# gaozhitong/MultiShiftSeg

Measured on AMD Instinct MI355X. Metric: train images/sec (DeepLabV3+ WRN38, fwd + RelContrastiveLoss + bwd + Adam), higher is better.
Workload: dtype f32; 1 GPU; c3: 2 images (1 orig+aug pair(s)) of 1024x2048 per GPU, stage-2 trainable set, train-mode BN/Dropout2d on the frozen trunk; images_per_gpu=2, height=1024, width=2048, stage=2, parallelism=dp1, rccl_ranks=0, loss_pairing=device, loss_sync=local

## Files before the change

### multishiftseg_amd/csrc/conv_wgrad.hip

```cpp
#include "mss_epilogue.h"
#include "wgrad_route.h"
static_assert(MSS_WGRAD_PERIMG_TAIL_BYTES == (long long)TN_PERIMG_MAX_SLOTS * 128 * 128 * 4, "include/mss_hip.h and tn_perimg_plan.h disagree");
#include <stdlib.h>

bool mss_wgrad_tn_bf16x3_eligible(const MssConvArgs& p, int lddy);
long long mss_wgrad_tn_bf16x3_ws_bytes(const MssConvArgs& p, int Cp);
void mss_wgrad_tn_bf16x3_plan(const MssConvArgs& p, WgradRoute& r);
int mss_wgrad_tn_bf16x3_launch(const MssConvArgs& p, const float* dy, int lddy, float* dwp, int Cp, float* ws, long long ws_bytes, void* stream);
int mss_stem7_wgrad_launch(const WgradRoute& r, const MssConvArgs& p, const float* dy, int lddy, float* dwp, float* ws, hipStream_t stream);

namespace {

constexpr int NT = 256;

template <int BKO, int BCI, int BP, int WK>
__global__ __launch_bounds__(NT) void conv_wgrad_kernel(MssConvArgs p, const float* __restrict__ dy, int lddy,
                                                        float* __restrict__ dwp, int Cp, int pix_per_split) {
  constexpr int LDA = BKO + 4;
  constexpr int LDB = BCI + 4;
  constexpr int WC = 4 / WK;
  constexpr int WTK = BKO / WK, WTC = BCI / WC;
  constexpr int TM = WTK / 32, TN = WTC / 32;
  constexpr int A_CPR = BKO / 4, B_CPR = BCI / 4;
  constexpr bool A_PART = BP * A_CPR < NT;
// ... 439 lines not shown
  };
  f32x16 acc[2][TNJ];
  auto zero_acc = [&]() {
#pragma unroll
    for (int i = 0; i < 2; ++i)
#pragma unroll
      for (int j = 0; j < TNJ; ++j)
#pragma unroll
        for (int q = 0; q < 16; ++q) acc[i][j][q] = 0.f;
  };
  auto mfma_chunk = [&](int set) {
#pragma unroll
    for (int s2 = 0; s2 < 4; ++s2)
#pragma unroll
      for (int i = 0; i < 2; ++i)
#pragma unroll
        for (int j = 0; j < TNJ; ++j)
          acc[i][j] = __builtin_amdgcn_mfma_f32_32x32x2f32(fa[set][i][s2], fb[set][j][s2], acc[i][j], 0, 0, 0);
  };
  auto epilogue = [&](long long w) {
    const int ct = (int)(w % ctiles); w /= ctiles;
    const int kt = (int)(w % ktiles); w /= ktiles;
    float* o = dst + (size_t)w * Kpad * Cp;
    const int colq = lane & 31, rowq = 4 * (lane >> 5);
#pragma unroll
    for (int j = 0; j < TNJ; ++j) {
      const int col = ct * BC + wn * (BC / 2) + j * 32 + colq;
      if (col >= Cp) continue;
#pragma unroll
      for (int i = 0; i < 2; ++i)
#pragma unroll
        for (int q = 0; q < 16; ++q) {
          const int row = kt * 128 + wm * 64 + i * 32 + (q & 3) + 8 * (q >> 2) + rowq;
          if (row < Kpad) o[(size_t)row * Cp + col] = acc[i][j][q];
        }
    }
  };

  long long cur = ld_w;
  int steps_left;
  {
    long long w = cur / ((long long)ktiles * ctiles);
    const int sp = (int)(w / P);
    const int t0 = sp * t_per_split;
    steps_left = (min(T, t0 + t_per_split) - t0 + 15) / 16;
  }
  setup(ld_w);
  issue_loads();
  finish_store(0);
  advance();
  zero_acc();
  __syncthreads();
  load_frags(0, 0, 0);
  int buf = 0;
  while (true) {
    issue_loads();
    load_frags(1, buf, 1);
    finish_store(buf ^ 1);
    advance();
    mfma_chunk(0);
    __syncthreads();
    load_frags(0, buf ^ 1, 0);
    mfma_chunk(1);
    buf ^= 1;
    if (--steps_left == 0) {
      epilogue(cur);
      cur += stride;
      if (cur >= total) break;
      zero_acc();
      long long w = cur / ((long long)ktiles * ctiles);
      const int sp = (int)(w / P);
      const int t0 = sp * t_per_split;
      steps_left = (min(T, t0 + t_per_split) - t0 + 15) / 16;
    }
  }
}

__global__ __launch_bounds__(256) void wgrad_reduce_kernel(const float* __restrict__ ws, float* __restrict__ dwp,
                                                           long long slab4, int splits) {
  const f32x4* w4 = reinterpret_cast<const f32x4*>(ws);
  f32x4* d4 = reinterpret_cast<f32x4*>(dwp);
  for (long long i = (long long)blockIdx.x * blockDim.x + threadIdx.x; i < slab4;
       i += (long long)gridDim.x * blockDim.x) {
    f32x4 a = w4[i];
    int sp = 1;
    for (; sp + 8 <= splits; sp += 8) {
      f32x4 v[8];
#pragma unroll
      for (int u = 0; u < 8; ++u) v[u] = w4[(long long)(sp + u) * slab4 + i];
#pragma unroll
      for (int u = 0; u < 8; ++u) a += v[u];
    }
    for (; sp < splits; ++sp) a += w4[(long long)sp * slab4 + i];
    d4[i] = a;
  }
}

template <int G>
__global__ __launch_bounds__(256) void wgrad_reduce_par_kernel(const float* __restrict__ ws, float* __restrict__ dwp, long long slab4,
                                                               int splits) {
  constexpr int EPB = 256 / G;
  __shared__ f32x4 part[G][EPB];
  const f32x4* w4 = reinterpret_cast<const f32x4*>(ws);
  const int el = threadIdx.x % EPB, g = threadIdx.x / EPB;
  const long long i = (long long)blockIdx.x * EPB + el;
  f32x4 a = {0.f, 0.f, 0.f, 0.f};
  if (i < slab4) {
    int sp = g;
    for (; sp + 3 * G < splits; sp += 4 * G) {
      const f32x4 v0 = w4[(long long)sp * slab4 + i], v1 = w4[(long long)(sp + G) * slab4 + i];
      const f32x4 v2 = w4[(long long)(sp + 2 * G) * slab4 + i], v3 = w4[(long long)(sp + 3 * G) * slab4 + i];
      a += v0; a += v1; a += v2; a += v3;
    }
    for (; sp < splits; sp += G) a += w4[(long long)sp * slab4 + i];
  }
  part[g][el] = a;
  __syncthreads();
  if (g == 0 && i < slab4) {
    f32x4 t = part[0][el];
#pragma unroll
    for (int k = 1; k < G; ++k) t += part[k][el];
    reinterpret_cast<f32x4*>(dwp)[i] = t;
  }
}

inline void launch_wgrad_reduce(const float* ws, float* dwp, long long slab4, int splits, int G, hipStream_t stream) {
  if (G == 1) {
    long long blocks = (slab4 + 255) / 256;
    if (blocks > 4096) blocks = 4096;
    hipLaunchKernelGGL(wgrad_reduce_kernel, dim3((int)blocks), dim3(256), 0, stream, ws, dwp, slab4, splits);
    return;
  }
#define RED(G_) hipLaunchKernelGGL(wgrad_reduce_par_kernel<G_>, dim3((unsigned)((slab4 + 256 / G_ - 1) / (256 / G_))), dim3(256), 0, stream, ws, dwp, slab4, splits)
  switch (G) {
    case 2: RED(2); break;
    case 4: RED(4); break;
    case 8: RED(8); break;
    case 16: RED(16); break;
    default: RED(32); break;
  }
#undef RED
}

typedef float f32x2 __attribute__((ext_vector_type(2)));
__device__ const float tn_zero_row[4096] = {0.f};
template <bool AFFINE = false, bool PERIMG = false>
__global__ __launch_bounds__(256, 1) void gemm_tn_direct_kernel(const float* __restrict__ A, const float* __restrict__ B,
                                                                float* __restrict__ out, int P, int M, int K, int C, long long a_bs,
                                                                long long b_bs, int Kpad, int Cp, int ktiles, int ctiles, int splits,
                                                                int tps, long long total, long long full, float* __restrict__ tail_ws,
                                                                const float* __restrict__ scale = nullptr,
                                                                const float* __restrict__ shift = nullptr, int relu = 0, int lda = 0,
                                                                const int* __restrict__ k_steps = nullptr, int k_base = 0,
                                                                int k_imgs = 1, int pi_slots = 0) {
  if (lda <= 0) lda = K;
  constexpr int KB = 4;
  constexpr int TND = 8;
  const int lane = threadIdx.x & 63, wave = threadIdx.x >> 6;
  long long t;
  int sp = 0, nsp = 1;
  long long tail_tile = -1, ntail = 0;
  int ct, kt, pb;
  if (PERIMG && pi_slots > 0) {
    const TnPerimgPlan pl = tn_perimg_plan(P / k_imgs, k_imgs, ktiles, ctiles, k_base, k_steps, pi_slots, M, tail_ws != nullptr);
    const int nwg = (int)((pl.total + 3) / 4), nrun = pl.tail ? (int)(pl.full / 4) : nwg;
    const int bid = (int)blockIdx.x;
    if (bid >= nwg) return;
    const long long job = (long long)(bid < nrun ? mss_xcd_remap(bid, nrun) : bid) * 4 + __builtin_amdgcn_readfirstlane(wave);
    TnPerimgJob jb;
    if (!tn_perimg_decode(pl, k_steps, job, jb)) return;
    ct = jb.ct; kt = jb.kt; pb = jb.pos * k_imgs + jb.img;
    if (jb.tail_tile >= 0) { sp = jb.sp; nsp = pl.splits; tail_tile = jb.tail_tile; ntail = pl.tail; tps = pl.tps; }
  } else {
    const long long job = (long long)(PERIMG ? mss_xcd_remap((int)blockIdx.x, (int)gridDim.x) : (int)blockIdx.x) * 4 + wave;
    if (job >= total) return;
    t = job;
    if (full >= 0) {
      if (job >= full) {
        ntail = (total - full) / splits;
        sp = (int)((job - full) / ntail);
        tail_tile = (job - full) - (long long)sp * ntail;
        t = full + tail_tile;
        nsp = splits;
      }
    } else {
      nsp = splits;
    }
    ct = (int)(t % ctiles); t /= ctiles;
    kt = (int)(t % ktiles); t /= ktiles;
    if (full >= 0) pb = (int)t;
    else { sp = (int)(t % splits); pb = (int)(t / splits); }
  }
  const int half = lane >> 5, j = lane & 31;
  const int r0 = nsp > 1 ? sp * tps : 0, r1 = nsp > 1 ? (r0 + tps < M ? r0 + tps : M) : M;
  const float* a = A + (size_t)pb * a_bs + (size_t)(kt * (32 * KB) + KB * j);
  const float* b = B + (size_t)pb * b_bs + (size_t)(ct * 128 + 4 * j);
  size_t b_ld = (size_t)C;
  if (PERIMG) {
    const int cend = 16 * (k_base + k_steps[pb % k_imgs]);
    if (ct * 128 >= cend) return;
    if (ct * 128 + 4 * j >= cend) { b = tn_zero_row + 4 * j; b_ld = 0; }
  }
  f32x16 acc[KB][4];
#pragma unroll
  for (int i = 0; i < KB; ++i)
#pragma unroll
    for (int q = 0; q < 4; ++q)
#pragma unroll
      for (int r = 0; r < 16; ++r) acc[i][q][r] = 0.f;
  f32x4 a0[TND], a1[TND];
  f32x4 b0[TND], b1[TND];
  const int last = r1 - 1;
  const float* az = tn_zero_row + (kt * (32 * KB) + KB * j);
  auto fetch = [&](int row, f32x4& va, f32x4& vb) {
    const bool ok = row <= last;
    const size_t rr = (size_t)(ok ? row : last);
    va = *reinterpret_cast<const f32x4*>(ok ? a + rr * lda : az);
    vb = *reinterpret_cast<const f32x4*>(b + rr * (PERIMG ? b_ld : (size_t)C));
  };
  f32x4 sc = {1.f, 1.f, 1.f, 1.f}, sh = {0.f, 0.f, 0.f, 0.f};
  if (AFFINE) {
    if (scale) sc = *reinterpret_cast<const f32x4*>(scale + ct * 128 + 4 * j);
    if (shift) sh = *reinterpret_cast<const f32x4*>(shift + ct * 128 + 4 * j);
  }
  const float fl = relu ? 0.f : -__builtin_huge_valf();
  auto compute = [&](const f32x4 (&va)[TND], const f32x4 (&vb)[TND]) {
#pragma unroll
    for (int d = 0; d < TND; ++d) {
      const f32x4 ca = va[d];
      f32x4 cb = vb[d];
      if (AFFINE) {
        cb = cb * sc + sh;
        cb.x = fmaxf(cb.x, fl); cb.y = fmaxf(cb.y, fl); cb.z = fmaxf(cb.z, fl); cb.w = fmaxf(cb.w, fl);
      }
#pragma unroll
      for (int i = 0; i < KB; ++i)
#pragma unroll
        for (int q = 0; q < 4; ++q) acc[i][q] = __builtin_amdgcn_mfma_f32_32x32x2f32(ca[i], cb[q], acc[i][q], 0, 0, 0);
    }
  };
#pragma unroll
  for (int d = 0; d < TND; ++d) fetch(r0 + 2 * d + half, a0[d], b0[d]);
  for (int r = r0; r < r1; r += 4 * TND) {
#pragma unroll
    for (int d = 0; d < TND; ++d) fetch(r + 2 * TND + 2 * d + half, a1[d], b1[d]);
    __builtin_amdgcn_sched_barrier(0);
    compute(a0, b0);
    __builtin_amdgcn_sched_barrier(0);
#pragma unroll
    for (int d = 0; d < TND; ++d) fetch(r + 4 * TND + 2 * d + half, a0[d], b0[d]);
    __builtin_amdgcn_sched_barrier(0);
    compute(a1, b1);
    __builtin_amdgcn_sched_barrier(0);
  }
  float* o;
  size_t ostride;
  if (tail_tile >= 0) {
    o = tail_ws + ((size_t)sp * ntail + tail_tile) * (128 * 128) + (size_t)(4 * j);
    ostride = 128;
  } else {
    o = out + ((size_t)(full >= 0 ? 0 : sp) * P + pb) * Kpad * Cp + (size_t)(kt * (32 * KB)) * Cp + (size_t)(ct * 128 + 4 * j);
    ostride = Cp;
  }
#pragma unroll
  for (int i = 0; i < KB; ++i)
#pragma unroll
    for (int r = 0; r < 16; ++r) {
      const int m = (r & 3) + 8 * (r >> 2) + 4 * half;
      const f32x4 v = {acc[i][0][r], acc[i][1][r], acc[i][2][r], acc[i][3][r]};
      *reinterpret_cast<f32x4*>(o + (size_t)(KB * m + i) * ostride) = v;
    }
}

__global__ __launch_bounds__(256) void tn_tail_reduce_kernel(const float* __restrict__ tail_ws, float* __restrict__ dwp, long long full,
                                                             long long ntail, int splits, int ktiles, int ctiles, int Kpad, int Cp) {
  const long long ti = blockIdx.x / 16;
  const int part = blockIdx.x % 16;
  long long t = full + ti;
  const int ct = (int)(t % ctiles); t /= ctiles;
  const int kt = (int)(t % ktiles); t /= ktiles;
  const int pb = (int)t;
  const int e = part * 1024 + threadIdx.x * 4;
  const int row = e >> 7, col = e & 127;
  const float* src = tail_ws + (size_t)ti * (128 * 128) + e;
  f32x4 a = *reinterpret_cast<const f32x4*>(src);
  for (int sp = 1; sp < splits; ++sp) a += *reinterpret_cast<const f32x4*>(src + (size_t)sp * ntail * (128 * 128));
  *reinterpret_cast<f32x4*>(dwp + (size_t)pb * Kpad * Cp + (size_t)(kt * 128 + row) * Cp + ct * 128 + col) = a;
}

__global__ __launch_bounds__(256) void tn_tail_reduce_perimg_kernel(const float* __restrict__ tail_ws, float* __restrict__ dwp, int P,
                                                                    int k_imgs, int ktiles, int ctiles, int k_base,
                                                                    const int* __restrict__ k_steps, int slots, int rows, int Kpad,
                                                                    int Cp) {
  const int ti = blockIdx.x / 16, part = blockIdx.x % 16;
  const TnPerimgPlan pl = tn_perimg_plan(P, k_imgs, ktiles, ctiles, k_base, k_steps, slots, rows, 1);
  if (ti >= pl.tail) return;
  TnPerimgJob jb;
  if (!tn_perimg_decode(pl, k_steps, pl.full + ti, jb)) return;
  const int pb = jb.pos * k_imgs + jb.img;
  const int e = part * 1024 + threadIdx.x * 4;
  const int row = e >> 7, col = e & 127;
  const float* src = tail_ws + (size_t)ti * (128 * 128) + e;
  f32x4 a = *reinterpret_cast<const f32x4*>(src);
  for (int sp = 1; sp < pl.splits; ++sp) a += *reinterpret_cast<const f32x4*>(src + (size_t)sp * pl.tail * (128 * 128));
  *reinterpret_cast<f32x4*>(dwp + (size_t)pb * Kpad * Cp + (size_t)(jb.kt * 128 + row) * Cp + jb.ct * 128 + col) = a;
}

__device__ float tn_zeros_rt[64];
template <int KB2, bool AFFINE>
__global__ __launch_bounds__(256, 2) void gemm_tn_narrow_kernel(const float* __restrict__ A, int lda, const float* __restrict__ B, int ldb,
                                                                const float* __restrict__ scale, const float* __restrict__ shift,
                                                                int relu, float* __restrict__ out, int M, int K, int Kpad, int Cp,
                                                                int ctiles, int tps, long long total) {
  typedef typename std::conditional<KB2 == 2, f32x2, float>::type avec;
  constexpr int TND = 8;
  const int lane = threadIdx.x & 63, wave = threadIdx.x >> 6;
  const long long job = (long long)blockIdx.x * 4 + wave;
  if (job >= total) return;
  const int ct = (int)(job % ctiles), sp = (int)(job / ctiles);
  const int half = lane >> 5, j = lane & 31;
  const int r0 = sp * tps, r1 = r0 + tps < M ? r0 + tps : M;
  const bool a_ok = KB2 * j + KB2 - 1 < K;
  const float* a = A + KB2 * j;
  const float* b = B + (size_t)(ct * 128 + 4 * j);
  f32x4 sc = {1.f, 1.f, 1.f, 1.f}, sh = {0.f, 0.f, 0.f, 0.f};
  if (AFFINE) {
    if (scale) sc = *reinterpret_cast<const f32x4*>(scale + ct * 128 + 4 * j);
    if (shift) sh = *reinterpret_cast<const f32x4*>(shift + ct * 128 + 4 * j);
  }
  const float fl = relu ? 0.f : -__builtin_huge_valf();
  f32x16 acc[KB2][4];
#pragma unroll
  for (int i = 0; i < KB2; ++i)
#pragma unroll
    for (int q = 0; q < 4; ++q)
#pragma unroll
      for (int r = 0; r < 16; ++r) acc[i][q][r] = 0.f;
  avec a0[TND], a1[TND];
  f32x4 b0[TND], b1[TND];
  const int last = r1 - 1;
  auto fetch = [&](int row, avec& va, f32x4& vb) {
    const bool ok = row <= last;
    const size_t rr = (size_t)(ok ? row : last);
    va = *reinterpret_cast<const avec*>((ok && a_ok) ? a + rr * lda : tn_zeros_rt);
    vb = *reinterpret_cast<const f32x4*>(b + rr * ldb);
  };
  auto compute = [&](const avec (&va)[TND], const f32x4 (&vb)[TND]) {
#pragma unroll
    for (int d = 0; d < TND; ++d) {
      f32x4 cb = vb[d];
      if (AFFINE) {
        cb = cb * sc + sh;
        cb.x = fmaxf(cb.x, fl); cb.y = fmaxf(cb.y, fl); cb.z = fmaxf(cb.z, fl); cb.w = fmaxf(cb.w, fl);
      }
#pragma unroll
      for (int i = 0; i < KB2; ++i) {
        float ai;
        if constexpr (KB2 == 2) ai = va[d][i]; else ai = va[d];
#pragma unroll
        for (int q = 0; q < 4; ++q) acc[i][q] = __builtin_amdgcn_mfma_f32_32x32x2f32(ai, cb[q], acc[i][q], 0, 0, 0);
      }
    }
  };
#pragma unroll
  for (int d = 0; d < TND; ++d) fetch(r0 + 2 * d + half, a0[d], b0[d]);
  for (int r = r0; r < r1; r += 4 * TND) {
#pragma unroll
    for (int d = 0; d < TND; ++d) fetch(r + 2 * TND + 2 * d + half, a1[d], b1[d]);
    __builtin_amdgcn_sched_barrier(0);
    compute(a0, b0);
    __builtin_amdgcn_sched_barrier(0);
#pragma unroll
    for (int d = 0; d < TND; ++d) fetch(r + 4 * TND + 2 * d + half, a0[d], b0[d]);
    __builtin_amdgcn_sched_barrier(0);
    compute(a1, b1);
    __builtin_amdgcn_sched_barrier(0);
  }
  float* o = out + (size_t)sp * Kpad * Cp + (size_t)(ct * 128 + 4 * j);
#pragma unroll
  for (int i = 0; i < KB2; ++i)
#pragma unroll
    for (int r = 0; r < 16; ++r) {
      const int k = KB2 * ((r & 3) + 8 * (r >> 2) + 4 * half) + i;
      const f32x4 v = {acc[i][0][r], acc[i][1][r], acc[i][2][r], acc[i][3][r]};
      if (k < Kpad) *reinterpret_cast<f32x4*>(o + (size_t)k * Cp) = v;
    }
}


inline int finish_splits(const WgradRoute& r, const MssConvArgs& p, int Cp, const float* ws, float* dwp, hipStream_t stream) {
  if (r.splits > 1) launch_wgrad_reduce(ws, dwp, (long long)r.positions * p.Kpad * Cp / 4, r.splits, r.reduce_group, stream);
  return mss_launch_status();
}

template <int BKO, int WK>
int launch_wgrad_conv(const WgradRoute& r, const MssConvArgs& p, const float* dy, int lddy, float* dwp, int Cp, float* ws, hipStream_t stream) {
  constexpr int BCI = 128, BP = 16;
  const size_t smem = (size_t)2 * BP * (BKO + 4 + BCI + 4) * sizeof(float);
  auto kern = conv_wgrad_kernel<BKO, BCI, BP, WK>;
  hipLaunchKernelGGL(kern, dim3(r.ktiles * r.ctiles, r.positions, r.splits), dim3(NT), smem, stream, p, dy, lddy,
                     r.splits > 1 ? ws : dwp, Cp, r.rows_per_split);
  return finish_splits(r, p, Cp, ws, dwp, stream);
}

int launch_wgrad_narrow(const WgradRoute& r, const MssConvArgs& p, const float* dy, int lddy, float* dwp, int Cp, float* ws, hipStream_t stream) {
  float* out = r.splits > 1 ? ws : dwp;
  const bool aff = wg_has_prologue(p);
  const dim3 grid((unsigned)((r.total + 3) / 4));
#define NARROW(KB2_, AFF_)                                                                                                          \
  hipLaunchKernelGGL((gemm_tn_narrow_kernel<KB2_, AFF_>), grid, dim3(256), 0, stream, dy, lddy, p.x, p.ldx, p.in_scale, p.in_shift,  \
                     p.in_relu, out, p.M, p.K, p.Kpad, Cp, r.ctiles, r.rows_per_split, r.total)
  if (p.K <= 32) { if (aff) NARROW(1, true); else NARROW(1, false); }
  else { if (aff) NARROW(2, true); else NARROW(2, false); }
#undef NARROW
  return finish_splits(r, p, Cp, ws, dwp, stream);
}

void launch_tn_direct(const WgradRoute& r, const MssConvArgs& p, long long jobs, const float* dy, int lddy, float* out, int Cp,
                      float* tail_ws, int slots, hipStream_t stream) {
  const bool perimg = p.k_steps != nullptr, aff = wg_has_prologue(p);
  const long long a_bs = p.batch > 1 ? p.y_bs : 0, b_bs = p.batch > 1 ? p.x_bs : 0;
  auto kern = perimg ? gemm_tn_direct_kernel<false, true> : aff ? gemm_tn_direct_kernel<true, false> : gemm_tn_direct_kernel<false, false>;
  hipLaunchKernelGGL(kern, dim3((unsigned)((jobs + 3) / 4)), dim3(256), 0, stream, dy, p.x, out, r.positions, p.M, p.K, p.C, a_bs, b_bs,
                     p.Kpad, Cp, r.ktiles, r.ctiles, r.splits, r.rows_per_split, jobs, r.full, tail_ws, aff ? p.in_scale : (const float*)nullptr,
                     aff ? p.in_shift : (const float*)nullptr, aff ? p.in_relu : 0, lddy, p.k_steps, p.k_base, p.k_imgs, slots);
}

int launch_wgrad_tn_direct(const WgradRoute& r, const MssConvArgs& p, const float* dy, int lddy, float* dwp, int Cp, float* ws, hipStream_t stream) {
  if (r.full >= 0) {
    const long long ntail = (r.total - r.full) / r.splits;
    launch_tn_direct(r, p, r.total, dy, lddy, dwp, Cp, ws, 0, stream);
    hipLaunchKernelGGL(tn_tail_reduce_kernel, dim3((unsigned)(ntail * 16)), dim3(256), 0, stream, ws, dwp, r.full, ntail, r.splits,
                       r.ktiles, r.ctiles, p.Kpad, Cp);
    return mss_launch_status();
  }
  launch_tn_direct(r, p, r.total, dy, lddy, r.splits > 1 ? ws : dwp, Cp, nullptr, 0, stream);
  return finish_splits(r, p, Cp, ws, dwp, stream);
}

int launch_wgrad_tn_perimg(const WgradRoute& r, const MssConvArgs& p, const float* dy, int lddy, float* dwp, int Cp, float* ws,
                           long long ws_bytes, const WgradSwitches& sw, hipStream_t stream) {
  if (sw.perimg_pack != 0 && p.k_imgs <= TN_PERIMG_MAX_IMGS) {
    int slots = sw.tn_slots / 32 * 32;
    slots = slots < 32 ? 32 : slots > TN_PERIMG_MAX_SLOTS ? TN_PERIMG_MAX_SLOTS : slots;
    const int P = p.batch / p.k_imgs;
    const bool tail = sw.tn_tail != 0 && ws && ws_bytes >= (long long)slots * (128 * 128 * 4) && r.total > slots;
    const long long jobs = tn_perimg_worst_jobs(P, p.k_imgs, r.ktiles, r.ctiles, slots, tail);
    launch_tn_direct(r, p, jobs, dy, lddy, dwp, Cp, tail ? ws : nullptr, slots, stream);
    if (tail)
      hipLaunchKernelGGL(tn_tail_reduce_perimg_kernel, dim3((unsigned)(slots / 2 * 16)), dim3(256), 0, stream, ws, dwp, P, p.k_imgs, r.ktiles,
                         r.ctiles, p.k_base, p.k_steps, slots, p.M, p.Kpad, Cp);
    return mss_launch_status();
  }
  launch_tn_direct(r, p, r.total, dy, lddy, dwp, Cp, nullptr, 0, stream);
  return mss_launch_status();
}

int launch_wgrad_tn_lds(const WgradRoute& r, const MssConvArgs& p, const float* dy, float* dwp, int Cp, float* ws, hipStream_t stream) {
  const bool wide = r.kernel == WG_TN_WIDE;
  const long long a_bs = p.batch > 1 ? p.y_bs : 0, b_bs = p.batch > 1 ? p.x_bs : 0;
  const size_t smem = (size_t)4 * TN_BT * TN_LD * sizeof(float);
  MssKernelInfo ki;
  if (int rc = mss_kernel_info<gemm_tn_wgrad_kernel>(NT, smem, 3, &ki)) return rc;
  const long long slots = (long long)(wide ? 2 : ki.occ > 3 ? 3 : ki.occ) * ki.cus;
  const int grid = (int)(r.total < slots ? r.total : slots);
  float* out = r.splits > 1 ? ws : dwp;
  if (wide) {
    const size_t smem2 = (size_t)2 * (128 + 256) * TN2_LDK * sizeof(float);
    hipLaunchKernelGGL(gemm_tn2_wgrad_kernel, dim3(grid), dim3(NT), smem2, stream, dy, p.x, out, r.positions, p.M, p.K, p.C, a_bs,
                       b_bs, p.Kpad, Cp, r.ktiles, r.ctiles, r.splits, r.rows_per_split, r.total);
  } else {
    hipLaunchKernelGGL(gemm_tn_wgrad_kernel, dim3(grid), dim3(NT), smem, stream, dy, p.x, out, r.positions, p.M, p.K, p.C, a_bs,
                       b_bs, p.Kpad, Cp, r.ktiles, r.ctiles, r.splits, r.rows_per_split, r.total);
  }
  return finish_splits(r, p, Cp, ws, dwp, stream);
}

const WgradSplitBf16 split_bf16 = {mss_wgrad_tn_bf16x3_eligible, mss_wgrad_tn_bf16x3_ws_bytes, mss_wgrad_tn_bf16x3_plan};

WgradSwitches wgrad_switches() {
  WgradSwitches sw;
  sw.tn = MSS_ENV_INT("MSS_WGRAD_TN", 5);
  sw.tn_affine = MSS_ENV_INT("MSS_WGRAD_TN_AFFINE", 1);
  sw.tn_tail = MSS_ENV_INT("MSS_WGRAD_TN_TAIL", 1);
  sw.narrow = MSS_ENV_INT("MSS_WGRAD_NARROW", 1);
  sw.perimg_pack = MSS_ENV_INT("MSS_WGRAD_PERIMG_PACK", 1);
  sw.tn_slots = MSS_ENV_INT("MSS_WGRAD_TN_SLOTS", TN_PERIMG_MAX_SLOTS);
  return sw;
}

int launch_route(const WgradRoute& r, const MssConvArgs& p, const float* dy, int lddy, float* dwp, int Cp, float* ws, long long ws_bytes,
                 const WgradSwitches& sw, hipStream_t s) {
  if (r.ws_bytes > 0 && (!ws || ws_bytes < r.ws_bytes)) return MSS_ERR_BAD_ARG;
  switch (r.kernel) {
    case WG_TN_BF16X3: return mss_wgrad_tn_bf16x3_launch(p, dy, lddy, dwp, Cp, ws, ws_bytes, s);
    case WG_TN_DIRECT_PERIMG: return launch_wgrad_tn_perimg(r, p, dy, lddy, dwp, Cp, ws, ws_bytes, sw, s);
    case WG_TN_DIRECT:
    case WG_TN_DIRECT_TAIL: return launch_wgrad_tn_direct(r, p, dy, lddy, dwp, Cp, ws, s);
    case WG_TN_WIDE:
    case WG_TN_LDS: return launch_wgrad_tn_lds(r, p, dy, dwp, Cp, ws, s);
    case WG_NARROW: return launch_wgrad_narrow(r, p, dy, lddy, dwp, Cp, ws, s);
    case WG_CONV_32: return launch_wgrad_conv<32, 1>(r, p, dy, lddy, dwp, Cp, ws, s);
    case WG_CONV_64: return launch_wgrad_conv<64, 2>(r, p, dy, lddy, dwp, Cp, ws, s);
    case WG_CONV_128: return launch_wgrad_conv<128, 2>(r, p, dy, lddy, dwp, Cp, ws, s);
    case WG_STEM7: return mss_stem7_wgrad_launch(r, p, dy, lddy, dwp, ws, s);
    case WG_TWO_PART: break;
  }
  return MSS_ERR_BAD_ARG;
}

}

void mss_wgrad_reduce_launch(const float* ws, float* dwp, long long slab4, int splits, hipStream_t stream) {
  launch_wgrad_reduce(ws, dwp, slab4, splits, wg_reduce_group(slab4, splits), stream);
}

extern "C" {

int mss_conv2d_wgrad_route(const MssConvArgs* args, int lddy) {
  MssConvArgs p = *args;
  p.M = p.N * p.OH * p.OW;
  if (p.M <= 0 || wg_stem7_form(p, 4)) return 0;
  const WgradSwitches sw = wgrad_switches();
  WgradFacts f;
  f.dense_dy = lddy == p.K;
  WgradRoute r = wgrad_route(p, lddy, p.C, f, sw, split_bf16);
  if (r.kernel == WG_TWO_PART) { f.dense_dy = false; r = wgrad_route(wgrad_part(p, r.wide_K, false), lddy, p.C, f, sw, split_bf16); }
  return r.kernel == WG_TN_BF16X3 ? 1 : 0;
}

long long mss_conv2d_wgrad_workspace_bytes(const MssConvArgs* args, int Cp) {
  MssConvArgs p = *args;
  p.M = p.N * p.OH * p.OW;
  if (p.M <= 0) return 0;
  if (wg_stem7_form(p, Cp)) return wg_plan_stem7(p).ws_bytes;
  return wgrad_workspace_bytes(p, Cp, wgrad_switches(), split_bf16);
}

int mss_conv2d_wgrad_f32(MssConvArgs* args, const float* dy, int lddy, float* dwp, int Cp, float* ws,
                         long long ws_bytes, void* stream) {
  const WgradSwitches sw = wgrad_switches();
  WgradCall c;
  if (const int rc = wgrad_resolve(args, dy, lddy, dwp, Cp, ws_bytes, sw, split_bf16, c)) return rc;
  if (c.empty) return MSS_OK;
  hipStream_t s = static_cast<hipStream_t>(stream);
  if (c.route.kernel != WG_TWO_PART) return launch_route(c.route, c.p, dy, lddy, dwp, Cp, ws, ws_bytes, sw, s);
  const int wide = c.route.wide_K;
  const int rc = launch_route(c.part_route[0], c.part[0], dy, lddy, dwp, Cp, ws, ws_bytes, sw, s);
  if (rc != MSS_OK) return rc;
  return launch_route(c.part_route[1], c.part[1], dy + wide, lddy, dwp + (size_t)wide * Cp, Cp, ws, ws_bytes, sw, s);
}

int mss_conv2d_wgrad_plan(const MssConvArgs* args, const float* dy, int lddy, const float* dwp, int Cp, long long ws_bytes, int part,
                          MssWgradPlan* out) {
  if (!args || !out || part < 0 || part > 2) return MSS_ERR_BAD_ARG;
  WgradCall c;
  if (const int rc = wgrad_resolve(args, dy, lddy, dwp, Cp, ws_bytes, wgrad_switches(), split_bf16, c)) return rc;
  MssWgradPlan o = {-1, 0, 0, 0, 0, 0, 0, 0, 0, 0, 0};
  if (!c.empty) {
    if (part != 0 && c.route.kernel != WG_TWO_PART) return MSS_ERR_BAD_ARG;
    const WgradRoute& r = part == 0 ? c.route : c.part_route[part - 1];
    o.kernel = r.kernel; o.ktiles = r.ktiles; o.ctiles = r.ctiles; o.positions = r.positions; o.splits = r.splits;
    o.rows_per_split = r.rows_per_split; o.total = r.total; o.full = r.full; o.ws_bytes = r.ws_bytes; o.wide_K = r.wide_K;
    o.reduce_group = r.reduce_group;
  } else if (part != 0) {
    return MSS_ERR_BAD_ARG;
  }
  *out = o;
  return MSS_OK;
}

}
```

### multishiftseg_amd/csrc/tn_perimg_plan.h

```cpp
#pragma once

#if !defined(__HIPCC__) && !defined(__host__)
#define __host__
#define __device__
#endif

#define TN_PERIMG_MAX_IMGS 64
#define TN_PERIMG_MAX_SLOTS 1024

struct TnPerimgPlan {
  int ktiles, ctiles, k_imgs, k_base, rows;
  int S;
  long long live;
  long long full;
  long long total;
  int tail;
  int splits, tps;
};

struct TnPerimgJob {
  int pos, img, kt, ct;
  int sp;
  int tail_tile;
  int r0, r1;
};

__host__ __device__ static inline int tn_perimg_ctiles(int k_base, int k_steps_n, int ctiles) {
  const int cols = 16 * (k_base + k_steps_n);
  int L = cols > 0 ? (cols + 127) / 128 : 0;
  return L < ctiles ? L : ctiles;
}

__host__ __device__ static inline TnPerimgPlan tn_perimg_plan(int P, int k_imgs, int ktiles, int ctiles, int k_base, const int* k_steps,
                                                              int slots, int rows, int want_tail) {
  TnPerimgPlan pl;
  pl.ktiles = ktiles; pl.ctiles = ctiles; pl.k_imgs = k_imgs; pl.k_base = k_base; pl.rows = rows;
  int sum = 0;
  for (int n = 0; n < k_imgs; ++n) sum += tn_perimg_ctiles(k_base, k_steps[n], ctiles);
  pl.S = ktiles * sum;
  pl.live = (long long)P * pl.S;
  pl.full = pl.live; pl.total = pl.live; pl.tail = 0; pl.splits = 1; pl.tps = rows;
  if (!want_tail || pl.live <= slots || pl.live % slots == 0) return pl;
  const long long rounds = (pl.live + slots - 1) / slots * slots;
  if (pl.live * 20 >= rounds * 19) return pl;
  const int tail = (int)(pl.live % slots);
  int ts = slots / tail;
  const int max_splits = (rows + 255) / 256;
  if (ts > max_splits) ts = max_splits;
  if (ts > 16) ts = 16;
  if (ts < 2) return pl;
  pl.tail = tail;
  pl.full = pl.live - tail;
  pl.tps = ((rows + ts - 1) / ts + 1) / 2 * 2;
  pl.splits = (rows + pl.tps - 1) / pl.tps;
  pl.total = pl.full + (long long)tail * pl.splits;
  return pl;
}

__host__ __device__ static inline bool tn_perimg_decode(const TnPerimgPlan& pl, const int* k_steps, long long job, TnPerimgJob& j) {
  if (job < 0 || job >= pl.total) return false;
  long long t = job;
  j.sp = 0; j.tail_tile = -1;
  if (job >= pl.full) {
    j.sp = (int)((job - pl.full) / pl.tail);
    j.tail_tile = (int)((job - pl.full) - (long long)j.sp * pl.tail);
    t = pl.full + j.tail_tile;
  }
  j.pos = (int)(t / pl.S);
  int rem = (int)(t - (long long)j.pos * pl.S);
  j.img = 0; j.kt = 0; j.ct = 0;
  for (int n = 0; n < pl.k_imgs; ++n) {
    const int L = tn_perimg_ctiles(pl.k_base, k_steps[n], pl.ctiles);
    const int g = pl.ktiles * L;
    if (rem < g) { j.img = n; j.kt = rem / L; j.ct = rem - j.kt * L; break; }
    rem -= g;
  }
  j.r0 = j.tail_tile >= 0 ? j.sp * pl.tps : 0;
  j.r1 = j.tail_tile >= 0 && j.r0 + pl.tps < pl.rows ? j.r0 + pl.tps : pl.rows;
  return true;
}

__host__ __device__ static inline long long tn_perimg_worst_jobs(int P, int k_imgs, int ktiles, int ctiles, int slots, int want_tail) {
  const long long worst = (long long)P * k_imgs * ktiles * ctiles;
  return worst + (want_tail && worst > slots ? slots : 0);
}
```

### multishiftseg_amd/csrc/wgrad_route.h

```cpp
#pragma once
#include <stdint.h>

#include "../../include/mss_hip.h"
#include "mss_gemm_dims.h"
#include "tn_perimg_plan.h"

struct WgradSwitches {
  int tn = 5;
  int tn_affine = 1;
  int tn_tail = 1;
  int narrow = 1;
  int perimg_pack = 1;
  int tn_slots = TN_PERIMG_MAX_SLOTS;
};

enum WgradKernel {
  WG_CONV_32 = MSS_WG_CONV_32,
  WG_CONV_64 = MSS_WG_CONV_64,
  WG_CONV_128 = MSS_WG_CONV_128,
  WG_NARROW = MSS_WG_NARROW,
  WG_TN_LDS = MSS_WG_TN_LDS,
  WG_TN_WIDE = MSS_WG_TN_WIDE,
  WG_TN_DIRECT = MSS_WG_TN_DIRECT,
  WG_TN_DIRECT_TAIL = MSS_WG_TN_DIRECT_TAIL,
  WG_TN_DIRECT_PERIMG = MSS_WG_TN_DIRECT_PERIMG,
  WG_TN_BF16X3 = MSS_WG_TN_BF16X3,
  WG_TWO_PART = MSS_WG_TWO_PART,
  WG_STEM7 = MSS_WG_STEM7,
};

struct WgradRoute {
  WgradKernel kernel = WG_CONV_128;
  int ktiles = 0, ctiles = 0;
  int positions = 1;
  int splits = 1;
  int rows_per_split = 0;
  long long total = 0;
  long long full = -1;
  long long ws_bytes = 0;
  int wide_K = 0;
  int reduce_group = 0;
};

struct WgradFacts {
  bool dense_dy = true;
  bool dy8 = true;
  bool x16 = true;
  bool affine16 = true;
};

struct WgradSplitBf16 {
  bool (*eligible)(const MssConvArgs& p, int lddy) = nullptr;
  long long (*ws_bytes)(const MssConvArgs& p, int Cp) = nullptr;
  void (*plan)(const MssConvArgs& p, WgradRoute& r) = nullptr;
};

static inline int wg_cdiv(long long a, long long b) { return (int)((a + b - 1) / b); }

static inline int split_search(long long base_jobs, int slots, int max_splits) {
  int splits = 1;
  double best = 0.0;
  for (int sp = 1; sp <= max_splits; ++sp) {
    const long long total = base_jobs * sp;
    const double eff = (double)total / (double)(((total + slots - 1) / slots) * slots);
    if (eff > best + 1e-9) { best = eff; splits = sp; }
    if (eff >= 0.95 && total >= slots) break;
  }
  return splits;
}

static inline int wg_positions(const MssConvArgs& p) { return p.batch > 1 ? p.batch : 1; }
static inline bool wg_has_prologue(const MssConvArgs& p) { return p.in_scale || p.in_shift || p.in_relu; }
static inline void wg_cut_rows(WgradRoute& r, int M, int splits, int granule) {
  r.rows_per_split = wg_cdiv(wg_cdiv(M, splits), granule) * granule;
  r.splits = wg_cdiv(M, r.rows_per_split);
}
static inline long long wg_slab_bytes(const WgradRoute& r, const MssConvArgs& p, int Cp) {
  return r.splits > 1 ? (long long)r.splits * r.positions * p.Kpad * Cp * 4 : 0;
}
static inline int wg_reduce_group(long long slab4, int splits) {
  int G = 1;
  while (G < 32 && slab4 * G < 65536 && splits >= 8 * G) G *= 2;
  return G;
}
static inline void wg_plan_slabs(WgradRoute& r, const MssConvArgs& p, int Cp) {
  r.ws_bytes = wg_slab_bytes(r, p, Cp);
  r.reduce_group = r.splits > 1 ? wg_reduce_group((long long)r.positions * p.Kpad * Cp / 4, r.splits) : 0;
}

static inline WgradRoute wg_plan_conv(const MssConvArgs& p, int Cp) {
  WgradRoute r;
  r.kernel = p.K <= 32 ? WG_CONV_32 : p.K <= 64 ? WG_CONV_64 : WG_CONV_128;
  const int bko = p.K <= 32 ? 32 : p.K <= 64 ? 64 : 128, bp = 16;
  r.ktiles = wg_cdiv(p.K, bko); r.ctiles = wg_cdiv(p.C, 128); r.positions = p.batch > 1 ? p.batch : p.R * p.S;
  const int base = r.ktiles * r.ctiles * r.positions;
  int max_splits = wg_cdiv(p.M, bp * 8);
  if (max_splits > 1024) max_splits = 1024;
  if (max_splits < 1) max_splits = 1;
  wg_cut_rows(r, p.M, split_search(base, 768, max_splits), bp);
  r.total = (long long)base * r.splits;
  wg_plan_slabs(r, p, Cp);
  return r;
}

static inline bool wg_narrow_eligible(const MssConvArgs& p, int lddy, int Cp, WgradFacts f, const WgradSwitches& sw) {
  if (sw.narrow == 0) return false;
  if (p.R * p.S != 1 || p.stride != 1 || p.pad != 0 || p.batch > 1 || p.OH != p.H || p.OW != p.W) return false;
  if (p.K > 64 || (p.K > 32 && p.K % 2) || p.C % 128 || Cp != p.C || p.ldx % 4) return false;
  if ((p.in_scale || p.in_shift) && p.in_ss_stride != 0) return false;
  if (p.M < 16384) return false;
  if (p.K > 32 && (lddy % 2 || !f.dy8)) return false;
  return f.x16 && ((!p.in_scale && !p.in_shift) || f.affine16);
}
static inline WgradRoute wg_plan_narrow(const MssConvArgs& p, int Cp) {
  WgradRoute r;
  r.kernel = WG_NARROW;
  r.ktiles = 1; r.ctiles = p.C / 128;
  int splits = (p.K <= 32 ? 3072 : 2048) / r.ctiles;
  const int max_splits = wg_cdiv(p.M, 512);
  if (splits > max_splits) splits = max_splits;
  if (splits < 1) splits = 1;
  wg_cut_rows(r, p.M, splits, 2);
  r.total = (long long)r.ctiles * r.splits;
  wg_plan_slabs(r, p, Cp);
  return r;
}

static inline WgradRoute wg_plan_tn_lds(const MssConvArgs& p, int Cp, bool wide) {
  WgradRoute r;
  r.kernel = wide ? WG_TN_WIDE : WG_TN_LDS;
  r.ktiles = wg_cdiv(p.K, 128); r.ctiles = wg_cdiv(p.C, wide ? 256 : 128); r.positions = wg_positions(p);
  const long long base = (long long)r.positions * r.ktiles * r.ctiles;
  int max_splits = wg_cdiv(p.M, 16 * 8);
  const int cap = p.batch > 1 ? 64 : 256;
  if (max_splits > cap) max_splits = cap;
  if (max_splits < 1) max_splits = 1;
  wg_cut_rows(r, p.M, split_search(base, wide ? 512 : 768, max_splits), 16);
  r.total = base * r.splits;
  wg_plan_slabs(r, p, Cp);
  return r;
}
static inline bool wg_tn_wide(const MssConvArgs& p, int Cp, const WgradSwitches& sw) {
  if (sw.tn == 4) return p.C % 256 == 0;
  if (sw.tn < 5 || p.C % 256) return false;
  const WgradRoute w = wg_plan_tn_lds(p, Cp, true);
  const double eff = (double)w.total / (double)(((w.total + 511) / 512) * 512);
  return w.splits == 1 && w.total >= 1024 && eff >= 0.9;
}

static inline WgradRoute wg_plan_tn_direct(const MssConvArgs& p, int Cp, const WgradSwitches& sw) {
  WgradRoute r;
  r.kernel = WG_TN_DIRECT;
  r.ktiles = p.K / 128; r.ctiles = p.C / 128; r.positions = wg_positions(p);
  const long long base = (long long)r.positions * r.ktiles * r.ctiles;
  const int slots = 1024;
  int max_splits = wg_cdiv(p.M, 256);
  if (sw.tn_tail != 0 && base > slots && base % slots != 0 && (double)base / (double)(((base + slots - 1) / slots) * slots) < 0.95) {
    const long long tail = base % slots;
    int ts = (int)(slots / tail);
    if (ts > max_splits) ts = max_splits;
    if (ts > 16) ts = 16;
    if (ts >= 2) {
      r.kernel = WG_TN_DIRECT_TAIL;
      r.full = base - tail;
      wg_cut_rows(r, p.M, ts, 2);
      r.total = r.full + tail * r.splits;
// ... 192 lines not shown
```

Measured before the change: 23.72 images/s.

## Stream-K chunking of per-image TN wgrad tail tiles across all workgroups

Adds a chunked tail mode to the per-image packed TN direct wgrad kernel. When the leftover tiles are too few to split evenly, their combined K-row stream is divided into equal chunks across all workgroup slots. Each wave may process two pieces that straddle tiles, writing partial sums into a workspace slot. A reworked tail reduce kernel then adds those partials onto the directly written first piece. The aim is to balance the last partial wave of tiles so the GPU is not left mostly idle at the end, at the cost of extra workspace traffic and a read-modify-write reduce.

```diff
diff --git a/multishiftseg_amd/csrc/conv_wgrad.hip b/multishiftseg_amd/csrc/conv_wgrad.hip
--- a/multishiftseg_amd/csrc/conv_wgrad.hip
+++ b/multishiftseg_amd/csrc/conv_wgrad.hip
@@ -615,27 +615,30 @@
                                                                 const float* __restrict__ scale = nullptr,
                                                                 const float* __restrict__ shift = nullptr, int relu = 0, int lda = 0,
                                                                 const int* __restrict__ k_steps = nullptr, int k_base = 0,
-                                                                int k_imgs = 1, int pi_slots = 0) {
+                                                                int k_imgs = 1, int pi_slots = 0, int pi_tail = 0) {
   if (lda <= 0) lda = K;
   constexpr int KB = 4;
   constexpr int TND = 8;
   const int lane = threadIdx.x & 63, wave = threadIdx.x >> 6;
+  const bool packed = PERIMG && pi_slots > 0;
+  TnPerimgPlan pl;
+  long long pjob = 0;
+  if (packed) {
+    const int bid = (int)blockIdx.x;
+    const long long live = (long long)(P / k_imgs) * tn_perimg_live(k_imgs, ktiles, ctiles, k_base, k_steps);
+    if ((long long)bid * 4 >= live + (tail_ws ? pi_slots : 0)) return;
+    pl = tn_perimg_plan(P / k_imgs, k_imgs, ktiles, ctiles, k_base, k_steps, pi_slots, M, tail_ws ? pi_tail : 0);
+    const int nwg = (int)((pl.total + 3) / 4), nrun = pl.tail ? (int)(pl.full / 4) : nwg;
+    if (bid >= nwg) return;
+    pjob = (long long)(bid < nrun ? mss_xcd_remap(bid, nrun) : bid) * 4 + __builtin_amdgcn_readfirstlane(wave);
+  }
   long long t;
   int sp = 0, nsp = 1;
   long long tail_tile = -1, ntail = 0;
-  int ct, kt, pb;
-  if (PERIMG && pi_slots > 0) {
-    const TnPerimgPlan pl = tn_perimg_plan(P / k_imgs, k_imgs, ktiles, ctiles, k_base, k_steps, pi_slots, M, tail_ws != nullptr);
-    const int nwg = (int)((pl.total + 3) / 4), nrun = pl.tail ? (int)(pl.full / 4) : nwg;
-    const int bid = (int)blockIdx.x;
-    if (bid >= nwg) return;
-    const long long job = (long long)(bid < nrun ? mss_xcd_remap(bid, nrun) : bid) * 4 + __builtin_amdgcn_readfirstlane(wave);
-    TnPerimgJob jb;
-    if (!tn_perimg_decode(pl, k_steps, job, jb)) return;
-    ct = jb.ct; kt = jb.kt; pb = jb.pos * k_imgs + jb.img;
-    if (jb.tail_tile >= 0) { sp = jb.sp; nsp = pl.splits; tail_tile = jb.tail_tile; ntail = pl.tail; tps = pl.tps; }
-  } else {
-    const long long job = (long long)(PERIMG ? mss_xcd_remap((int)blockIdx.x, (int)gridDim.x) : (int)blockIdx.x) * 4 + wave;
+  int ct = 0, kt = 0, pb = 0, r0 = 0, r1 = 0, slot = -1;
+  if (!packed) {
+    const long long job = (long long)(PERIMG ? mss_xcd_remap((int)blockIdx.x, (int)gridDim.x) : (int)blockIdx.x) * 4 +
+                          (PERIMG ? __builtin_amdgcn_readfirstlane(wave) : wave);
     if (job >= total) return;
     t = job;
     if (full >= 0) {
@@ -653,15 +656,27 @@
     kt = (int)(t % ktiles); t /= ktiles;
     if (full >= 0) pb = (int)t;
     else { sp = (int)(t % splits); pb = (int)(t / splits); }
-  }
-  const int half = lane >> 5, j = lane & 31;
-  const int r0 = nsp > 1 ? sp * tps : 0, r1 = nsp > 1 ? (r0 + tps < M ? r0 + tps : M) : M;
+    r0 = nsp > 1 ? sp * tps : 0;
+    r1 = nsp > 1 ? (r0 + tps < M ? r0 + tps : M) : M;
+    if (PERIMG && ct * 128 >= 16 * (k_base + k_steps[pb % k_imgs])) return;
+  }
+  const int pieces = packed ? tn_perimg_pieces(pl, pjob) : 1;
+#pragma unroll 1
+  for (int piece = 0; piece < pieces; ++piece) {
+  if (packed) {
+    TnPerimgJob jb;
+    if (!tn_perimg_piece(pl, k_steps, pjob, piece, jb)) continue;
+    ct = jb.ct; kt = jb.kt; pb = jb.pos * k_imgs + jb.img;
+    r0 = jb.r0; r1 = jb.r1; slot = jb.slot;
+  }
+  int lane_p = lane;
+  if (PERIMG) asm volatile("" : "+v"(lane_p));
+  const int half = lane_p >> 5, j = lane_p & 31;
   const float* a = A + (size_t)pb * a_bs + (size_t)(kt * (32 * KB) + KB * j);
   const float* b = B + (size_t)pb * b_bs + (size_t)(ct * 128 + 4 * j);
   size_t b_ld = (size_t)C;
   if (PERIMG) {
     const int cend = 16 * (k_base + k_steps[pb % k_imgs]);
-    if (ct * 128 >= cend) return;
     if (ct * 128 + 4 * j >= cend) { b = tn_zero_row + 4 * j; b_ld = 0; }
   }
   f32x16 acc[KB][4];
@@ -718,7 +733,10 @@
   }
   float* o;
   size_t ostride;
-  if (tail_tile >= 0) {
+  if (slot >= 0) {
+    o = tail_ws + (size_t)slot * (128 * 128) + (size_t)(4 * j);
+    ostride = 128;
+  } else if (tail_tile >= 0) {
     o = tail_ws + ((size_t)sp * ntail + tail_tile) * (128 * 128) + (size_t)(4 * j);
     ostride = 128;
   } else {
@@ -733,6 +751,7 @@
       const f32x4 v = {acc[i][0][r], acc[i][1][r], acc[i][2][r], acc[i][3][r]};
       *reinterpret_cast<f32x4*>(o + (size_t)(KB * m + i) * ostride) = v;
     }
+  }
 }
 
 __global__ __launch_bounds__(256) void tn_tail_reduce_kernel(const float* __restrict__ tail_ws, float* __restrict__ dwp, long long full,
@@ -754,19 +773,29 @@
 __global__ __launch_bounds__(256) void tn_tail_reduce_perimg_kernel(const float* __restrict__ tail_ws, float* __restrict__ dwp, int P,
                                                                     int k_imgs, int ktiles, int ctiles, int k_base,
                                                                     const int* __restrict__ k_steps, int slots, int rows, int Kpad,
-                                                                    int Cp) {
-  const int ti = blockIdx.x / 16, part = blockIdx.x % 16;
-  const TnPerimgPlan pl = tn_perimg_plan(P, k_imgs, ktiles, ctiles, k_base, k_steps, slots, rows, 1);
-  if (ti >= pl.tail) return;
-  TnPerimgJob jb;
-  if (!tn_perimg_decode(pl, k_steps, pl.full + ti, jb)) return;
-  const int pb = jb.pos * k_imgs + jb.img;
-  const int e = part * 1024 + threadIdx.x * 4;
-  const int row = e >> 7, col = e & 127;
-  const float* src = tail_ws + (size_t)ti * (128 * 128) + e;
-  f32x4 a = *reinterpret_cast<const f32x4*>(src);
-  for (int sp = 1; sp < pl.splits; ++sp) a += *reinterpret_cast<const f32x4*>(src + (size_t)sp * pl.tail * (128 * 128));
-  *reinterpret_cast<f32x4*>(dwp + (size_t)pb * Kpad * Cp + (size_t)(jb.kt * 128 + row) * Cp + jb.ct * 128 + col) = a;
+                                                                    int Cp, int want_tail) {
+  const TnPerimgPlan pl = tn_perimg_plan(P, k_imgs, ktiles, ctiles, k_base, k_steps, slots, rows, want_tail);
+  for (int item = (int)blockIdx.x; item < pl.tail * 16; item += (int)gridDim.x) {
+    const int ti = item >> 4, part = item & 15;
+    TnPerimgJob jb;
+    tn_perimg_tile(pl, k_steps, pl.full + ti, jb);
+    const int pb = jb.pos * k_imgs + jb.img;
+    const int e = part * 1024 + threadIdx.x * 4;
+    const int row = e >> 7, col = e & 127;
+    float* dst = dwp + (size_t)pb * Kpad * Cp + (size_t)(jb.kt * 128 + row) * Cp + jb.ct * 128 + col;
+    f32x4 a;
+    if (pl.chunk) {
+      int first, last;
+      tn_perimg_chunks_of(pl, ti, first, last);
+      a = *reinterpret_cast<const f32x4*>(dst);
+      for (int k = first; k < last; ++k) a += *reinterpret_cast<const f32x4*>(tail_ws + (size_t)(4 * k + (ti & 3)) * (128 * 128) + e);
+    } else {
+      const float* src = tail_ws + (size_t)ti * (128 * 128) + e;
+      a = *reinterpret_cast<const f32x4*>(src);
+      for (int sp = 1; sp < pl.splits; ++sp) a += *reinterpret_cast<const f32x4*>(src + (size_t)sp * pl.tail * (128 * 128));
+    }
+    *reinterpret_cast<f32x4*>(dst) = a;
+  }
 }
 
 __device__ float tn_zeros_rt[64];
@@ -880,13 +909,13 @@
 }
 
 void launch_tn_direct(const WgradRoute& r, const MssConvArgs& p, long long jobs, const float* dy, int lddy, float* out, int Cp,
-                      float* tail_ws, int slots, hipStream_t stream) {
+                      float* tail_ws, int slots, hipStream_t stream, int pi_tail = 0) {
   const bool perimg = p.k_steps != nullptr, aff = wg_has_prologue(p);
   const long long a_bs = p.batch > 1 ? p.y_bs : 0, b_bs = p.batch > 1 ? p.x_bs : 0;
   auto kern = perimg ? gemm_tn_direct_kernel<false, true> : aff ? gemm_tn_direct_kernel<true, false> : gemm_tn_direct_kernel<false, false>;
   hipLaunchKernelGGL(kern, dim3((unsigned)((jobs + 3) / 4)), dim3(256), 0, stream, dy, p.x, out, r.positions, p.M, p.K, p.C, a_bs, b_bs,
                      p.Kpad, Cp, r.ktiles, r.ctiles, r.splits, r.rows_per_split, jobs, r.full, tail_ws, aff ? p.in_scale : (const float*)nullptr,
-                     aff ? p.in_shift : (const float*)nullptr, aff ? p.in_relu : 0, lddy, p.k_steps, p.k_base, p.k_imgs, slots);
+                     aff ? p.in_shift : (const float*)nullptr, aff ? p.in_relu : 0, lddy, p.k_steps, p.k_base, p.k_imgs, slots, pi_tail);
 }
 
 int launch_wgrad_tn_direct(const WgradRoute& r, const MssConvArgs& p, const float* dy, int lddy, float* dwp, int Cp, float* ws, hipStream_t stream) {
@@ -909,10 +938,11 @@
     const int P = p.batch / p.k_imgs;
     const bool tail = sw.tn_tail != 0 && ws && ws_bytes >= (long long)slots * (128 * 128 * 4) && r.total > slots;
     const long long jobs = tn_perimg_worst_jobs(P, p.k_imgs, r.ktiles, r.ctiles, slots, tail);
-    launch_tn_direct(r, p, jobs, dy, lddy, dwp, Cp, tail ? ws : nullptr, slots, stream);
+    const int want_tail = !tail ? 0 : sw.perimg_chunk != 0 ? 2 : 1;
+    launch_tn_direct(r, p, jobs, dy, lddy, dwp, Cp, tail ? ws : nullptr, slots, stream, want_tail);
     if (tail)
-      hipLaunchKernelGGL(tn_tail_reduce_perimg_kernel, dim3((unsigned)(slots / 2 * 16)), dim3(256), 0, stream, ws, dwp, P, p.k_imgs, r.ktiles,
-                         r.ctiles, p.k_base, p.k_steps, slots, p.M, p.Kpad, Cp);
+      hipLaunchKernelGGL(tn_tail_reduce_perimg_kernel, dim3((unsigned)slots), dim3(256), 0, stream, ws, dwp, P, p.k_imgs, r.ktiles,
+                         r.ctiles, p.k_base, p.k_steps, slots, p.M, p.Kpad, Cp, want_tail);
     return mss_launch_status();
   }
   launch_tn_direct(r, p, r.total, dy, lddy, dwp, Cp, nullptr, 0, stream);
@@ -949,6 +979,7 @@
   sw.narrow = MSS_ENV_INT("MSS_WGRAD_NARROW", 1);
   sw.perimg_pack = MSS_ENV_INT("MSS_WGRAD_PERIMG_PACK", 1);
   sw.tn_slots = MSS_ENV_INT("MSS_WGRAD_TN_SLOTS", TN_PERIMG_MAX_SLOTS);
+  sw.perimg_chunk = MSS_ENV_INT("MSS_WGRAD_PERIMG_CHUNK", 1);
   return sw;
 }
 
diff --git a/multishiftseg_amd/csrc/tn_perimg_plan.h b/multishiftseg_amd/csrc/tn_perimg_plan.h
--- a/multishiftseg_amd/csrc/tn_perimg_plan.h
+++ b/multishiftseg_amd/csrc/tn_perimg_plan.h
@@ -16,6 +16,7 @@
   long long total;
   int tail;
   int splits, tps;
+  int chunk, nchunk;
 };
 
 struct TnPerimgJob {
@@ -23,6 +24,7 @@
   int sp;
   int tail_tile;
   int r0, r1;
+  int slot;
 };
 
 __host__ __device__ static inline int tn_perimg_ctiles(int k_base, int k_steps_n, int ctiles) {
@@ -31,21 +33,38 @@
   return L < ctiles ? L : ctiles;
 }
 
+__host__ __device__ static inline int tn_perimg_live(int k_imgs, int ktiles, int ctiles, int k_base, const int* k_steps) {
+  int sum = 0;
+  for (int n = 0; n < k_imgs; ++n) sum += tn_perimg_ctiles(k_base, k_steps[n], ctiles);
+  return ktiles * sum;
+}
+
 __host__ __device__ static inline TnPerimgPlan tn_perimg_plan(int P, int k_imgs, int ktiles, int ctiles, int k_base, const int* k_steps,
                                                               int slots, int rows, int want_tail) {
   TnPerimgPlan pl;
   pl.ktiles = ktiles; pl.ctiles = ctiles; pl.k_imgs = k_imgs; pl.k_base = k_base; pl.rows = rows;
-  int sum = 0;
-  for (int n = 0; n < k_imgs; ++n) sum += tn_perimg_ctiles(k_base, k_steps[n], ctiles);
-  pl.S = ktiles * sum;
+  pl.S = tn_perimg_live(k_imgs, ktiles, ctiles, k_base, k_steps);
   pl.live = (long long)P * pl.S;
-  pl.full = pl.live; pl.total = pl.live; pl.tail = 0; pl.splits = 1; pl.tps = rows;
+  pl.full = pl.live; pl.total = pl.live; pl.tail = 0; pl.splits = 1; pl.tps = rows; pl.chunk = 0; pl.nchunk = 0;
   if (!want_tail || pl.live <= slots || pl.live % slots == 0) return pl;
   const long long rounds = (pl.live + slots - 1) / slots * slots;
   if (pl.live * 20 >= rounds * 19) return pl;
   const int tail = (int)(pl.live % slots);
   int ts = slots / tail;
   const int max_splits = (rows + 255) / 256;
+  if (ts < 2 && max_splits >= 2 && want_tail >= 2) {
+    const long long stream = (long long)((tail + 3) / 4) * rows;
+    const int wgs = slots / 4;
+    const long long c = ((stream + wgs - 1) / wgs + 1) / 2 * 2;
+    if (c > rows || stream + c > 0x7fffffffll) return pl;
+    pl.tail = tail;
+    pl.full = pl.live - tail;
+    pl.chunk = pl.tps = (int)c;
+    pl.nchunk = (int)((stream + c - 1) / c);
+    pl.splits = (rows + pl.chunk - 1) / pl.chunk + 1;
+    pl.total = pl.full + 4ll * pl.nchunk;
+    return pl;
+  }
   if (ts > max_splits) ts = max_splits;
   if (ts > 16) ts = 16;
   if (ts < 2) return pl;
@@ -57,15 +76,7 @@
   return pl;
 }
 
-__host__ __device__ static inline bool tn_perimg_decode(const TnPerimgPlan& pl, const int* k_steps, long long job, TnPerimgJob& j) {
-  if (job < 0 || job >= pl.total) return false;
-  long long t = job;
-  j.sp = 0; j.tail_tile = -1;
-  if (job >= pl.full) {
-    j.sp = (int)((job - pl.full) / pl.tail);
-    j.tail_tile = (int)((job - pl.full) - (long long)j.sp * pl.tail);
-    t = pl.full + j.tail_tile;
-  }
+__host__ __device__ static inline void tn_perimg_tile(const TnPerimgPlan& pl, const int* k_steps, long long t, TnPerimgJob& j) {
   j.pos = (int)(t / pl.S);
   int rem = (int)(t - (long long)j.pos * pl.S);
   j.img = 0; j.kt = 0; j.ct = 0;
@@ -75,9 +86,53 @@
     if (rem < g) { j.img = n; j.kt = rem / L; j.ct = rem - j.kt * L; break; }
     rem -= g;
   }
-  j.r0 = j.tail_tile >= 0 ? j.sp * pl.tps : 0;
-  j.r1 = j.tail_tile >= 0 && j.r0 + pl.tps < pl.rows ? j.r0 + pl.tps : pl.rows;
+}
+
+__host__ __device__ static inline bool tn_perimg_decode(const TnPerimgPlan& pl, const int* k_steps, long long job, TnPerimgJob& j) {
+  if (job < 0 || job >= pl.total || (pl.chunk && job >= pl.full)) return false;
+  long long t = job;
+  int sp = 0, tail_tile = -1, slot = -1;
+  if (job >= pl.full) {
+    sp = (int)((job - pl.full) / pl.tail);
+    tail_tile = (int)((job - pl.full) - (long long)sp * pl.tail);
+    slot = (int)(job - pl.full);
+    t = pl.full + tail_tile;
+  }
+  tn_perimg_tile(pl, k_steps, t, j);
+  const int r0 = tail_tile >= 0 ? sp * pl.tps : 0;
+  j.sp = sp; j.tail_tile = tail_tile;
+  j.r0 = r0;
+  j.r1 = tail_tile >= 0 && r0 + pl.tps < pl.rows ? r0 + pl.tps : pl.rows;
+  j.slot = slot;
   return true;
+}
+
+__host__ __device__ static inline int tn_perimg_pieces(const TnPerimgPlan& pl, long long job) { return pl.chunk && job >= pl.full ? 2 : 1; }
+
+__host__ __device__ static inline bool tn_perimg_piece(const TnPerimgPlan& pl, const int* k_steps, long long job, int piece, TnPerimgJob& j) {
+  if (!pl.chunk || job < pl.full) return piece == 0 && tn_perimg_decode(pl, k_steps, job, j);
+  if (job >= pl.total || piece < 0 || piece > 1) return false;
+  const int cj = (int)(job - pl.full);
+  const int wave = cj & 3;
+  const int s0 = (cj >> 2) * pl.chunk, end = (pl.tail + 3) / 4 * pl.rows;
+  const int s1 = s0 + pl.chunk < end ? s0 + pl.chunk : end;
+  const int quad = s0 / pl.rows + piece, q0 = quad * pl.rows;
+  const int tile = 4 * quad + wave;
+  if (s1 <= q0 || tile >= pl.tail) return false;
+  tn_perimg_tile(pl, k_steps, pl.full + tile, j);
+  const int r0 = piece ? 0 : s0 - q0;
+  j.sp = 0; j.tail_tile = tile;
+  j.r0 = r0;
+  j.r1 = s1 - q0 < pl.rows ? s1 - q0 : pl.rows;
+  j.slot = r0 == 0 ? -1 : cj;
+  return true;
+}
+
+__host__ __device__ static inline void tn_perimg_chunks_of(const TnPerimgPlan& pl, int tile, int& first, int& last) {
+  const int q0 = tile / 4 * pl.rows;
+  first = q0 / pl.chunk + 1;
+  last = (q0 + pl.rows + pl.chunk - 1) / pl.chunk;
+  if (last > pl.nchunk) last = pl.nchunk;
 }
 
 __host__ __device__ static inline long long tn_perimg_worst_jobs(int P, int k_imgs, int ktiles, int ctiles, int slots, int want_tail) {
diff --git a/multishiftseg_amd/csrc/wgrad_route.h b/multishiftseg_amd/csrc/wgrad_route.h
--- a/multishiftseg_amd/csrc/wgrad_route.h
+++ b/multishiftseg_amd/csrc/wgrad_route.h
@@ -12,6 +12,7 @@
   int narrow = 1;
   int perimg_pack = 1;
   int tn_slots = TN_PERIMG_MAX_SLOTS;
+  int perimg_chunk = 1;
 };
 
 enum WgradKernel {
```

Result: no change. 23.75 images/s (median of 6 runs) (+0.1%).
